# VIS4ROB-lab/covins

Measured on AMD Instinct MI355X. Metric: GBA iterations/sec, 5-agent EuRoC merged map, higher is better.
Workload: dtype f64

## Files before the change

covins_amd/csrc/nd_plan.hip:

```cpp
#include "nd_plan.hpp"

#include <algorithm>
#include <cstdint>
#include <cstdlib>
#include <queue>
#include <thread>
#include <tuple>

namespace covgpu {
namespace {

struct Builder {
  const int K;
  const bool vi;
  const int leaf_dims;
  const std::vector<std::vector<int>>& adj;
  const std::vector<int>& chain_of;
  NdHostPlan& out;
  std::vector<int> reg, deg;
  std::vector<int> side;
  std::vector<char> inS;
  int regid = 0;
  int top_mode = 0;
  double group_frac = 3.0;
// ... 109 lines not shown
              s1 += sd[pick] ? -size[pick] : size[pick]; sd[pick] ^= 1;
            }
            if (!balanced(s1, frac) || s1 == 0 || s1 == total) continue;
            if (best_w < 0 || w < best_w) { best_w = w; side_best.assign(sd.begin(), sd.end()); }
          }
      }
      if (nc <= kBruteChains) {
        if (best_w < 0) best = 2;
        side_best.assign(nc, 0);
        for (int c = 0; c < nc; ++c) side_best[c] = (char)(best >> c & 1);
      } else if (best_w < 0) {
        side_best.assign(nc, 0);
        side_best[(int)(std::max_element(size.begin(), size.end()) - size.begin())] = 1;
      }
      if (side_best[0]) for (auto& b : side_best) b ^= 1;
      for (int v : vars) side[v] = (int)side_best[side[v]];
    } else if (chains.size() >= 2) {
      nparts = (int)chains.size();
      for (int v : vars) side[v] = (int)(std::lower_bound(chains.begin(), chains.end(), chain_of[v >> 1]) - chains.begin());
    } else {
      std::vector<int> pos;
      for (int v : vars) pos.push_back(v >> 1);
      std::sort(pos.begin(), pos.end());
      pos.erase(std::unique(pos.begin(), pos.end()), pos.end());
      if (pos.size() < 2) { leaf(vars, parent); return; }
      const int m = pos[pos.size() / 2];
      for (int v : vars) side[v] = (v >> 1) >= m;
    }
    ++regid;
    for (int v : vars) { reg[v] = regid; inS[v] = 0; }
    std::priority_queue<std::tuple<int, int, int>> heap;
    for (int v : vars) {
      int d = 0;
      for (int w : adj[v]) d += (reg[w] == regid && side[w] != side[v]) ? 1 : 0;
      deg[v] = d;
      if (d) heap.push(std::make_tuple(d, 1 - (v & 1), -v));
    }
    std::vector<int> S;
    while (!heap.empty()) {
      const auto top = heap.top(); heap.pop();
      const int v = -std::get<2>(top);
      if (inS[v] || std::get<0>(top) != deg[v] || deg[v] == 0) continue;
      inS[v] = 1; S.push_back(v);
      for (int w : adj[v])
        if (reg[w] == regid && side[w] != side[v] && !inS[w] && deg[w] > 0) { if (--deg[w]) heap.push(std::make_tuple(deg[w], 1 - (w & 1), -w)); }
      deg[v] = 0;
    }
    for (size_t q = S.size(); q-- > 0;) {
      const int v = S[q];
      bool needed = false;
      for (int w : adj[v]) if (reg[w] == regid && side[w] != side[v] && !inS[w]) { needed = true; break; }
      if (!needed) { inS[v] = 0; S[q] = -1; }
    }
    S.erase(std::remove(S.begin(), S.end(), -1), S.end());
    std::vector<std::vector<int>> parts(nparts);
    for (int v : vars) if (!inS[v]) parts[side[v]].push_back(v);
    const int n = S.empty() ? parent : new_node(S, parent);
    for (auto& pt : parts) build(pt, n);
  }
};

}

static void nd_graph(int K, bool vi, int nchains, const int* chain_ptr, int npairs, const int* pair_i, const int* pair_j, int nepairs, const int* epair_i,
                     const int* epair_j, std::vector<std::vector<int>>& adj, std::vector<int>& chain_of) {
  chain_of.assign(K, 0);
  for (int c = 0; c < nchains; ++c) for (int q = chain_ptr[c]; q < chain_ptr[c + 1]; ++q) chain_of[q] = c;
  adj.assign(2 * (size_t)K, {});
  auto link = [&](int a, int b) { if (a != b) { adj[a].push_back(b); adj[b].push_back(a); } };
  for (int p = 0; p < npairs; ++p) link(2 * pair_i[p], 2 * pair_j[p]);
  for (int p = 0; p < nepairs; ++p) link(2 * epair_i[p], 2 * epair_j[p]);
  if (vi)
    for (int c = 0; c < nchains; ++c)
      for (int q = chain_ptr[c]; q < chain_ptr[c + 1]; ++q) {
        link(2 * q + 1, 2 * q);
        if (q > chain_ptr[c]) {
          const int v[4] = {2 * (q - 1), 2 * (q - 1) + 1, 2 * q, 2 * q + 1};
          for (int a = 0; a < 4; ++a) for (int b = a + 1; b < 4; ++b) link(v[a], v[b]);
        }
      }
  for (auto& a : adj) { std::sort(a.begin(), a.end()); a.erase(std::unique(a.begin(), a.end()), a.end()); }
}

static bool nd_plan_build_mode(int top_mode, double group_frac, int K, bool vi, const std::vector<std::vector<int>>& adj, const std::vector<int>& chain_of,
                               int leaf_dims, NdHostPlan& out) {
  out = NdHostPlan();
  out.K = K; out.vi = vi ? 1 : 0; out.nvar = 2 * K;
  out.vnode.assign(2 * (size_t)K, -1); out.voff.assign(2 * (size_t)K, 0); out.vord.assign(2 * (size_t)K, -1);
  if (K <= 0) return false;
  std::vector<int> all;
  for (int q = 0; q < K; ++q) { all.push_back(2 * q); if (vi) all.push_back(2 * q + 1); }
  Builder bld(K, vi, leaf_dims, adj, chain_of, out);
  bld.top_mode = top_mode; bld.group_frac = group_frac;
  bld.build(all, -1);
  const int nn = out.nnodes;
  auto is_proper_ancestor = [&](int a, int n) {
    if (out.depth[a] >= out.depth[n]) return false;
    while (out.depth[n] > out.depth[a]) n = out.parent[n];
    return n == a;
  };
  {
    std::vector<int> hgt(nn, 0);
    int nlev = 0;
    for (int n = nn - 1; n >= 0; --n) { for (int c : out.child[n]) hgt[n] = std::max(hgt[n], hgt[c] + 1); nlev = std::max(nlev, hgt[n] + 1); }
    auto panels = [](int d) { return std::max(1, (d + 255) / 256); };
    std::vector<int> levc(nlev, 1);
    for (int n = 0; n < nn; ++n) levc[hgt[n]] = std::max(levc[hgt[n]], panels(out.own_dims[n]));
    for (int l = 0; l + 1 < nlev; ++l) {
      const int m = levc[l];
      if (m < 2) continue;
      std::vector<std::pair<int, int>> moves;
      std::vector<int> extra(nn, 0);
      bool ok = true;
      for (int n = 0; n < nn && ok; ++n) {
        if (hgt[n] != l || panels(out.own_dims[n]) < m) continue;
        const int need = out.own_dims[n] - 256 * (m - 1);
        int cnt = 0, mv = 0;
        for (size_t q = out.own[n].size(); q-- > 0 && mv < need;) { mv += NdHostPlan::vdim(out.own[n][q]); ++cnt; }
        if (need > 64 || out.parent[n] < 0 || cnt >= (int)out.own[n].size()) { ok = false; break; }
        moves.emplace_back(n, cnt); extra[out.parent[n]] += mv;
      }
      for (int n = 0; n < nn && ok; ++n) if (extra[n] && panels(out.own_dims[n] + extra[n]) > levc[hgt[n]]) ok = false;
      if (!ok) continue;
      for (auto& mvp : moves) {
        const int n = mvp.first, pn = out.parent[n];
        std::vector<int> up(out.own[n].end() - mvp.second, out.own[n].end());
        out.own[n].resize(out.own[n].size() - mvp.second);
        for (int v : up) out.own[pn].push_back(v);
        for (int node : {n, pn}) {
          int off = 0, ord = 0;
          for (int v : out.own[node]) { out.vnode[v] = node; out.voff[v] = off; out.vord[v] = ord++; off += NdHostPlan::vdim(v); }
          out.own_dims[node] = off;
        }
      }
      levc[l] = m - 1;
    }
  }
  out.strct.assign(nn, {});
  out.st_dims.assign(nn, 0);
  std::vector<int> stamp(2 * (size_t)K, -1);
  for (int n = nn - 1; n >= 0; --n) {
    std::vector<int>& st = out.strct[n];
    auto add = [&](int w) { if (stamp[w] != n) { stamp[w] = n; st.push_back(w); } };
    for (int v : out.own[n])
      for (int w : adj[v]) {
        const int m = out.vnode[w];
        if (m == n) continue;
        if (is_proper_ancestor(m, n)) add(w);
        else if (!is_proper_ancestor(n, m)) return false;
      }
    for (int c : out.child[n])
      for (int w : out.strct[c]) if (out.vnode[w] != n) add(w);
    std::sort(st.begin(), st.end(), [&](int a, int b) {
      return std::make_pair(-out.depth[out.vnode[a]], out.vord[a]) < std::make_pair(-out.depth[out.vnode[b]], out.vord[b]);
    });
    int d = 0;
    for (int w : st) d += NdHostPlan::vdim(w);
    out.st_dims[n] = d;
  }
  out.level.assign(nn, 0); out.slot.assign(nn, 0);
  for (int n = nn - 1; n >= 0; --n)
    for (int c : out.child[n]) out.level[n] = std::max(out.level[n], out.level[c] + 1);
  out.nlev = 0; out.maxdepth = 0;
  for (int n = 0; n < nn; ++n) { out.nlev = std::max(out.nlev, out.level[n] + 1); out.maxdepth = std::max(out.maxdepth, out.depth[n] + 1); }
  out.lev_nodes.assign(out.nlev, {});
  for (int n = 0; n < nn; ++n) { out.slot[n] = (int)out.lev_nodes[out.level[n]].size(); out.lev_nodes[out.level[n]].push_back(n); }
  out.lev_nI.assign(out.nlev, 0); out.lev_nO.assign(out.nlev, 0); out.lev_ntot.assign(out.nlev, 0);
  for (int l = 0; l < out.nlev; ++l) {
    int mo = 0, ms = 0;
    for (int n : out.lev_nodes[l]) { mo = std::max(mo, out.own_dims[n]); ms = std::max(ms, out.st_dims[n]); }
    out.lev_nI[l] = std::max(256, ((mo + 255) / 256) * 256);
    out.lev_nO[l] = ((ms + 127) / 128) * 128;
    out.lev_ntot[l] = out.lev_nI[l] + out.lev_nO[l];
    out.front_elems += (size_t)out.lev_nodes[l].size() * out.lev_ntot[l] * out.lev_ntot[l];
  }
  for (int n = 0; n < nn; ++n) {
    const double m = out.own_dims[n], b = out.st_dims[n];
    out.flops += m * m * m / 3.0 + m * m * b + m * b * b;
  }
  return true;
}

static double nd_plan_cost(const NdHostPlan& hp) {
  double t = hp.flops / 30e12;
  for (int l = 0; l < hp.nlev; ++l) t += (hp.lev_nI[l] / 256) * 140e-6 + 40e-6;
  return t;
}

bool nd_plan_build(int K, bool vi, int nchains, const int* chain_ptr, int npairs, const int* pair_i, const int* pair_j, int nepairs,
                   const int* epair_i, const int* epair_j, int leaf_dims, NdHostPlan& out, int top_mode) {
  std::vector<std::vector<int>> adj;
  std::vector<int> chain_of;
  out = NdHostPlan();
  out.K = K; out.vi = vi ? 1 : 0; out.nvar = 2 * K;
  if (K <= 0) return false;
  nd_graph(K, vi, nchains, chain_ptr, npairs, pair_i, pair_j, nepairs, epair_i, epair_j, adj, chain_of);
  int forced = top_mode;
  if (const char* e = getenv("COVGPU_ND_TOP")) forced = atoi(e) != 0 ? 1 : 0;
  std::vector<int> modes, leaves;
  if (nchains < 3 || forced == 0 || leaf_dims >= (1 << 29)) modes = {0};
  else if (forced == 1) modes = {1};
  else modes = {0, 1};
  if (leaf_dims > 0) leaves = {leaf_dims};
  else leaves = {600, 400, 500, 900};
  std::vector<double> fracs = {3.0, 2.5};
  if (const char* e = getenv("COVGPU_ND_GROUP_FRAC")) fracs = {std::max(2.0, atof(e))};
  struct Cand { int mode, leaf; double frac; NdHostPlan hp; bool ok = false; double cost = 0; };
  std::vector<Cand> cand;
  for (int lf : leaves)
    for (int m : modes)
      for (double fr : (m == 1 ? fracs : std::vector<double>{3.0})) { cand.emplace_back(); cand.back().mode = m; cand.back().leaf = lf; cand.back().frac = fr; }
  auto run = [&](size_t i) {
    try {
      cand[i].ok = nd_plan_build_mode(cand[i].mode, cand[i].frac, K, vi, adj, chain_of, cand[i].leaf, cand[i].hp);
      if (cand[i].ok) cand[i].cost = nd_plan_cost(cand[i].hp);
    } catch (...) { cand[i].ok = false; }
  };
  if (cand.size() == 1) run(0);
  else {
    std::vector<std::thread> th;
    std::vector<char> started(cand.size(), 0);
    for (size_t i = 1; i < cand.size(); ++i) {
      try { th.emplace_back(run, i); started[i] = 1; } catch (...) { break; }
    }
    run(0);
    for (auto& t : th) t.join();
    for (size_t i = 1; i < cand.size(); ++i) if (!started[i]) run(i);
  }
  int best = -1;
  for (size_t i = 0; i < cand.size(); ++i) if (cand[i].ok && (best < 0 || cand[i].cost < cand[best].cost)) best = (int)i;
  if (best < 0) return false;
  out = std::move(cand[best].hp);
  out.top_mode = cand[best].mode; out.leaf = cand[best].leaf; out.group_frac100 = (int)(cand[best].frac * 100.0 + 0.5);
  return true;
}

double nd_shard_cost(const NdHostPlan& hp, int world) {
  const int nn = hp.nnodes;
  double chain = 0.0;
  for (int l = 0; l < hp.nlev; ++l) chain += (hp.lev_nI[l] / 256) * 140e-6 + 40e-6;
  if (hp.shard_policy == 1) {
    NdShardAcct a;
    nd_shard_account(hp, world, a);
    double busiest = 0.0;
    for (double f : a.rank_fl) busiest = std::max(busiest, f);
    constexpr double kCollLatency = 30e-6;
    return busiest / 30e12 + chain + (world > 1 ? 2.0 * (world - 1) / world * a.bytes / 150e9 + a.collectives * kCollLatency : 0.0);
  }
  double top_fl = 0.0, exch = 0.0;
  std::vector<double> rank_fl(std::max(world, 1), 0.0);
  for (int n = 0; n < nn; ++n) {
    const double m = hp.own_dims[n], b = hp.st_dims[n], fl = m * m * m / 3.0 + m * m * b + m * b * b;
    if (hp.node_rank.empty() || hp.node_rank[n] < 0) { top_fl += fl; exch += 0.5 * (m + b) * (m + b) * 8.0; }
    else rank_fl[hp.node_rank[n]] += fl;
  }
  double busiest = 0.0;
  for (double f : rank_fl) busiest = std::max(busiest, f);
  return (top_fl + busiest) / 30e12 + chain + (world > 1 ? 2.0 * (world - 1) / world * exch / 150e9 : 0.0);
}

static void nd_shard_grow(NdHostPlan& hp, int world, double top_cap_bytes, std::vector<char>& top, double top_bytes) {
  const int nn = hp.nnodes;
  hp.node_rank.assign(nn, -1);
  hp.nsub = 0;
  hp.world = world;
  std::vector<double> w(nn, 0.0), sub(nn, 0.0);
  for (int n = 0; n < nn; ++n) { const double m = hp.own_dims[n], b = hp.st_dims[n]; w[n] = m * m * m / 3.0 + m * m * b + m * b * b + 1.0; }
  for (int n = nn - 1; n >= 0; --n) { sub[n] += w[n]; if (hp.parent[n] >= 0) sub[hp.parent[n]] += sub[n]; }
  std::vector<int> cand;
  for (int n = 0; n < nn; ++n)
    if (top[n]) for (int c : hp.child[n]) if (!top[c]) cand.push_back(c);
  for (int it = 0; it < 256; ++it) {
    if (cand.empty()) break;
    std::sort(cand.begin(), cand.end(), [&](int a, int b) { return sub[a] != sub[b] ? sub[a] > sub[b] : a < b; });
    double tot = 0.0;
    for (int c : cand) tot += sub[c];
    if ((int)cand.size() >= world && sub[cand[0]] <= 1.25 * tot / world) break;
    int pick = -1;
    for (size_t q = 0; q < cand.size() && pick < 0; ++q) {
      const int c = cand[q];
      const double nb = 8.0 * (double)(hp.own_dims[c] + hp.st_dims[c]) * (double)(hp.own_dims[c] + hp.st_dims[c]);
      if (!hp.child[c].empty() && top_bytes + nb <= top_cap_bytes) pick = (int)q;
    }
    if (pick < 0) break;
    const int c = cand[pick];
    cand.erase(cand.begin() + pick);
    top[c] = 1; top_bytes += 8.0 * (double)(hp.own_dims[c] + hp.st_dims[c]) * (double)(hp.own_dims[c] + hp.st_dims[c]);
    for (int d : hp.child[c]) cand.push_back(d);
  }
  std::sort(cand.begin(), cand.end(), [&](int a, int b) { return sub[a] != sub[b] ? sub[a] > sub[b] : a < b; });
  std::vector<double> load(world, 0.0);
  std::vector<int> owner(nn, -1);
  for (int c : cand) {
    int best = 0;
    for (int r = 1; r < world; ++r) if (load[r] < load[best]) best = r;
    owner[c] = best; load[best] += sub[c];
  }
  hp.nsub = (int)cand.size();
  for (int n = 0; n < nn; ++n) {
    if (top[n]) { hp.node_rank[n] = -1; continue; }
    hp.node_rank[n] = owner[n] >= 0 ? owner[n] : hp.node_rank[hp.parent[n]];
  }
}

void nd_shard_assign(NdHostPlan& hp, int world, double top_cap_bytes) {
  hp.shard_policy = 0;
  std::vector<char> top(hp.nnodes, 0);
  double top_bytes = 0.0;
  for (int n = 0; n < hp.nnodes; ++n)
    if (hp.parent[n] < 0) { top[n] = 1; top_bytes += 8.0 * (double)hp.own_dims[n] * hp.own_dims[n]; }
  nd_shard_grow(hp, world, top_cap_bytes, top, top_bytes);
}

void nd_shard_assign_dist(NdHostPlan& hp, int world, double top_cap_bytes, int min_order) {
  hp.shard_policy = 1;
  const int nn = hp.nnodes;
  std::vector<char> top(nn, 0);
  for (int n = 0; n < nn; ++n)
    if (hp.parent[n] < 0 || hp.own_dims[n] + hp.st_dims[n] >= min_order)
      for (int a = n; a >= 0 && !top[a]; a = hp.parent[a]) top[a] = 1;
  double top_bytes = 0.0;
  for (int n = 0; n < nn; ++n) if (top[n]) top_bytes += 8.0 * (double)(hp.own_dims[n] + hp.st_dims[n]) * (double)(hp.own_dims[n] + hp.st_dims[n]);
  nd_shard_grow(hp, world, top_cap_bytes, top, top_bytes);
}

void nd_shard_account(const NdHostPlan& hp, int world, NdShardAcct& out) {
  const int nn = hp.nnodes;
  world = std::max(world, 1);
  out = NdShardAcct();
  out.rank_fl.assign(world, 0.0);
  const bool sh = !hp.node_rank.empty();
  auto is_top = [&](int n) { return !sh || hp.node_rank[n] < 0; };
  double top_own = 0.0, rhs_top = 0.0, tiles = 0.0;
  std::vector<int> toph(nn, 0);
  for (int n = nn - 1; n >= 0; --n) if (is_top(n)) for (int c : hp.child[n]) if (is_top(c)) toph[n] = std::max(toph[n], toph[c] + 1);
  std::vector<int> lev_panels;
  for (int n = 0; n < nn; ++n) {
    const double m = hp.own_dims[n], b = hp.st_dims[n];
    if (!is_top(n)) { out.rank_fl[hp.node_rank[n]] += m * m * m / 3.0 + m * m * b + m * b * b; continue; }
    top_own += m;
    const int nIr = (hp.own_dims[n] + 127) / 128, nO = (hp.st_dims[n] + 127) / 128, np = (hp.own_dims[n] + 255) / 256;
// ... 47 lines not shown
```

covins_amd/csrc/nd_plan.hpp:

```cpp
#pragma once
#include <cstdint>
#include <vector>

namespace covgpu {

struct NdHostPlan {
  int K = 0, vi = 0, nvar = 0;
  int nnodes = 0, nlev = 0, maxdepth = 0;
  std::vector<int> parent, depth, level, slot;
  std::vector<std::vector<int>> own, strct, child;
  std::vector<int> own_dims, st_dims;
  std::vector<int> vnode, voff, vord;
  std::vector<std::vector<int>> lev_nodes;
  std::vector<int> lev_nI, lev_nO, lev_ntot;
  std::vector<int> node_rank;
  int nsub = 0;
  int world = 0, shard_policy = 0;
  int top_mode = 0, leaf = 0, group_frac100 = 300;
  double flops = 0;
  size_t front_elems = 0;
  static int vdim(int v) { return (v & 1) ? 9 : 6; }
};

bool nd_plan_build(int K, bool vi, int nchains, const int* chain_ptr, int npairs, const int* pair_i, const int* pair_j, int nepairs,
                   const int* epair_i, const int* epair_j, int leaf_dims, NdHostPlan& out, int top_mode = -1);

void nd_shard_assign(NdHostPlan& hp, int world, double top_cap_bytes = 48.0 * 1048576.0);
void nd_shard_assign_dist(NdHostPlan& hp, int world, double top_cap_bytes = 48.0 * 1048576.0, int min_order = 4096);
inline int nd_tile_owner(int node, int q, int world) { return world > 0 ? (q + node) % world : 0; }
double nd_shard_cost(const NdHostPlan& hp, int world);
struct NdShardAcct { std::vector<double> rank_fl; double bytes = 0.0; int collectives = 0; };
void nd_shard_account(const NdHostPlan& hp, int world, NdShardAcct& out);
void nd_plan_remap(NdHostPlan& hp, const std::vector<int>& var_map);

}
```

covins_amd/csrc/solver.hip:

```cpp
#include <dlfcn.h>

#include <algorithm>
#include <atomic>
#include <chrono>
#include <condition_variable>
#include <memory>
#include <mutex>
#include <cmath>
#include <cstdio>
#include <cstdlib>
#include <cstring>
#include <string>
#include <thread>
#include <vector>

#include "common.hpp"
#include "nd_plan.hpp"

using namespace covgpu;

static thread_local std::string g_err;
extern "C" const char* covgpu_last_error(void) { return g_err.c_str(); }

#define HIPCHK(expr)                                                                            \
  do {                                                                                          \
    hipError_t e_ = (expr);                                                                     \
    if (e_ != hipSuccess) {                                                                     \
      g_err = std::string(#expr) + ": " + hipGetErrorString(e_);                                \
      return e_ == hipErrorOutOfMemory ? COVGPU_ERR_OUT_OF_MEMORY : COVGPU_ERR_NO_DEVICE;       \
    }                                                                                           \
  } while (0)

struct covgpu_profile_t {
  double t_build_ms = 0, t_factor_ms = 0, t_syrk_ms = 0, syrk_flops = 0;
  long n_build = 0, n_factor = 0, n_syrk = 0;
};

struct PlanCache {
  bool valid = false; int K = 0; bool vi = false; int leaf = 0;
  int top_env = -1; double frac_env = 0.0;
  std::vector<int> chain_ptr, pos_kf;
  std::vector<uint64_t> keys;
  NdHostPlan hp;
};

constexpr int COVGPU_ERR_GATE_TIMEOUT = -1000;
struct covgpu_group;
struct covgpu_context {
  int device = 0;
  hipStream_t st = nullptr;
  DevProblem P;
  bool have = false, pgo = false;
  std::vector<void*> allocs;
  size_t alloc_bytes = 0;
  double* h_scal = nullptr;
  double* h_tr = nullptr;
  double* h_box = nullptr;
  double* d_box = nullptr;
  double box_seq = 0.0;
  int profiling = 0;
  covgpu_profile_t prof;
  hipEvent_t ev[4] = {nullptr, nullptr, nullptr, nullptr};
  CholAux chol;
  PgoPlan pgo_plan;
  PlanCache plan_cache;
  NdDev nd;
  bool sharded = false;
  int rank = 0, world = 1;
  std::shared_ptr<NdHostPlan> shard_plan;
  struct Reducer* reducer = nullptr;
  double* d_red = nullptr;
  double cur_damp = 0.0;
  bool coll_failed = false;
  std::string coll_err;
  covgpu_group* group = nullptr;
  int* d_pairkey = nullptr;
  std::vector<int> h_perm;
  std::atomic<int>* peer_fail = nullptr;
};

struct Reducer {
  int rank = 0, world = 1;
  size_t calls = 0, bytes = 0;
  virtual ~Reducer() {}
  virtual int allreduce(double* dev, size_t n, int op, hipStream_t st) = 0;
  virtual void abort() {}
  virtual std::string last_error() { return "all-reduce failed"; }
};

struct GroupPtrs { double* p[16]; };
__global__ __launch_bounds__(256) void k_group_reduce(GroupPtrs g, int world, size_t n, int op, double* __restrict__ out) {
  for (size_t i = (size_t)blockIdx.x * 256 + threadIdx.x; i < n; i += (size_t)gridDim.x * 256) {
    double v = g.p[0][i];
    for (int r = 1; r < world; ++r) v = op == 0 ? v + g.p[r][i] : fmax(v, g.p[r][i]);
    out[i] = v;
  }
}
struct covgpu_group {
  int world = 1;
  std::mutex m; std::condition_variable cv; int count = 0; long gen = 0; bool broken = false;
  GroupPtrs ptrs;
  bool wait() {
    std::unique_lock<std::mutex> lk(m);
    const long g0 = gen;
    if (++count == world) { count = 0; ++gen; cv.notify_all(); return !broken; }
    cv.wait_for(lk, std::chrono::seconds(600), [&] { return gen != g0 || broken; });
    if (gen == g0) { broken = true; cv.notify_all(); return false; }
    return !broken;
  }
};
struct GroupReducer : Reducer {
  covgpu_group* g = nullptr;
  double* scratch = nullptr; size_t scratch_n = 0;
  ~GroupReducer() override { if (scratch) (void)hipFree(scratch); }
  void abort() override { std::lock_guard<std::mutex> lk(g->m); g->broken = true; g->cv.notify_all(); }
  std::string last_error() override { return "in-process group all-reduce failed (a member gave up, timed out, or the scratch allocation failed)"; }
  int allreduce(double* dev, size_t n, int op, hipStream_t st) override {
    if (n == 0) return 0;
    if (scratch_n < n) { if (scratch) (void)hipFree(scratch); if (hipMalloc((void**)&scratch, n * sizeof(double)) != hipSuccess) return 1; scratch_n = n; }
    (void)hipStreamSynchronize(st);
    { std::lock_guard<std::mutex> lk(g->m); g->ptrs.p[rank] = dev; }
    if (!g->wait()) return 1;
    hipLaunchKernelGGL(k_group_reduce, dim3((unsigned)std::min<size_t>((n + 255) / 256, 4096)), dim3(256), 0, st, g->ptrs, world, n, op, scratch);
// ... 371 lines not shown
    for (size_t h = 0; h < queue.size(); ++h) { const int u = queue[h]; for (int v : nb[u]) if (level[v] < 0) { level[v] = level[u] + 1; queue.push_back(v); } }
    return queue.back();
  };
  int pos = 0;
  for (int k = 0; k < K; ++k) {
    if (placed[k]) continue;
    const int far = bfs(k);
    for (int v : queue) level[v] = -1;
    bfs(far);
    for (int v : queue) { level[v] = -1; placed[v] = 1; perm[v] = pos; pos_kf[pos] = v; ++pos; }
    chain_ptr.push_back(pos);
  }
}

static bool host_pairs(const covgpu_problem* p, const std::vector<int>& perm, std::vector<int>& pi, std::vector<int>& pj, std::vector<int>& ei,
                       std::vector<int>& ej) {
  std::vector<long long> keys;
  for (int l = 0; l < p->num_lm; ++l)
    for (int a = p->lm_obs_ptr[l]; a < p->lm_obs_ptr[l + 1]; ++a) {
      if (p->kf_fixed[p->obs_kf[a]]) continue;
      for (int b = p->lm_obs_ptr[l]; b < p->lm_obs_ptr[l + 1]; ++b) {
        if (p->kf_fixed[p->obs_kf[b]]) continue;
        const int pa = perm[p->obs_kf[a]], pb = perm[p->obs_kf[b]];
        if (pb < pa) keys.push_back(((long long)pa << 32) | (unsigned)pb);
      }
    }
  std::sort(keys.begin(), keys.end()); keys.erase(std::unique(keys.begin(), keys.end()), keys.end());
  pi.resize(keys.size()); pj.resize(keys.size()); ei.clear(); ej.clear();
  for (size_t q = 0; q < keys.size(); ++q) { pi[q] = (int)(keys[q] >> 32); pj[q] = (int)(keys[q] & 0xffffffffll); }
  for (int e = 0; e < p->num_edge; ++e) {
    const int a = perm[p->edge_i[e]], b = perm[p->edge_j[e]];
    if (a == b) return false;
    ei.push_back(std::max(a, b)); ej.push_back(std::min(a, b));
  }
  return true;
}

static int nd_leaf_dims(int requested) {
  if (requested > 0) return requested;
  const char* e = getenv("COVGPU_ND_LEAF");
  const int v = e ? atoi(e) : 0;
  return v > 0 ? v : 0;
}
static int nd_plan_create_mode(const covgpu_options* opt, const covgpu_problem* p, int32_t leaf_dims, covgpu_nd_plan** out, int top_mode);
extern "C" int covgpu_nd_plan_create(const covgpu_options* opt, const covgpu_problem* p, int32_t leaf_dims, covgpu_nd_plan** out) { return nd_plan_create_mode(opt, p, leaf_dims, out, -1); }
static int nd_plan_create_mode(const covgpu_options* opt, const covgpu_problem* p, int32_t leaf_dims, covgpu_nd_plan** out, int top_mode) {
  return guarded([&] {
    const bool vi = !opt->visual_only;
    *out = nullptr;
    RC(validate(p, false, vi));
    std::vector<int> perm, pos_kf, chain_ptr, pi, pj, ei, ej;
    RC(build_chains(p, vi, perm, pos_kf, chain_ptr));
    if (!host_pairs(p, perm, pi, pj, ei, ej)) { g_err = "invalid problem: self edge"; return (int)COVGPU_ERR_INVALID_ARG; }
    covgpu_nd_plan* pl = new covgpu_nd_plan();
    pl->pos_kf = pos_kf;
    const auto t_pl = std::chrono::steady_clock::now();
    struct PT { std::chrono::steady_clock::time_point t0; ~PT() { if (getenv("COVGPU_PLAN_TIMING")) std::fprintf(stderr, "[covgpu] nd_plan_build %.1f ms\n", std::chrono::duration<double>(std::chrono::steady_clock::now() - t0).count() * 1e3); } } pt{t_pl};
    if (!nd_plan_build(p->num_kf, vi, (int)chain_ptr.size() - 1, chain_ptr.data(), (int)pi.size(), pi.data(), pj.data(), (int)ei.size(), ei.data(), ej.data(),
                       nd_leaf_dims(leaf_dims), pl->hp, top_mode)) {
      delete pl; g_err = "nested-dissection plan: a coupling joins two branches"; return (int)COVGPU_ERR_INVALID_ARG;
    }
    *out = pl;
    return (int)COVGPU_OK;
  });
}
extern "C" int covgpu_nd_plan_create_pgo(const covgpu_options* opt, const covgpu_problem* p, int32_t leaf_dims, covgpu_nd_plan** out) {
  (void)opt;
  return guarded([&] {
    *out = nullptr;
    RC(validate(p, true, false));
    std::vector<int> perm, pos_kf, chain_ptr;
    build_chains_pgo(p, perm, pos_kf, chain_ptr);
    std::vector<uint64_t> keys;
    for (int e = 0; e < p->num_edge; ++e) {
      const int a = perm[p->edge_i[e]], b = perm[p->edge_j[e]];
      if (a == b) { g_err = "invalid problem: self edge"; return (int)COVGPU_ERR_INVALID_ARG; }
      keys.push_back(((uint64_t)(uint32_t)std::max(a, b) << 32) | (uint32_t)std::min(a, b));
    }
    std::sort(keys.begin(), keys.end()); keys.erase(std::unique(keys.begin(), keys.end()), keys.end());
    std::vector<int> ei(keys.size()), ej(keys.size());
    for (size_t q = 0; q < keys.size(); ++q) { ei[q] = (int)(keys[q] >> 32); ej[q] = (int)(keys[q] & 0xffffffffull); }
    covgpu_nd_plan* pl = new covgpu_nd_plan();
    pl->pos_kf = pos_kf;
    if (!nd_plan_build(p->num_kf, false, (int)chain_ptr.size() - 1, chain_ptr.data(), 0, nullptr, nullptr, (int)ei.size(), ei.data(), ej.data(), nd_leaf_dims(leaf_dims), pl->hp, -1)) {
      delete pl; g_err = "nested-dissection plan: a coupling joins two branches"; return (int)COVGPU_ERR_INVALID_ARG;
    }
    *out = pl;
    return (int)COVGPU_OK;
  });
}
extern "C" void covgpu_nd_plan_destroy(covgpu_nd_plan* pl) { delete pl; }
extern "C" void covgpu_nd_plan_info(const covgpu_nd_plan* pl, int64_t* out) {
  for (int i = 0; i < 16; ++i) out[i] = 0;
  const NdHostPlan& h = pl->hp;
  out[0] = h.nnodes; out[1] = h.nlev; out[2] = h.maxdepth;
  for (int n = 0; n < h.nnodes; ++n) {
    out[3] += (int64_t)h.own[n].size(); out[4] += (int64_t)h.strct[n].size();
    out[7] = std::max<int64_t>(out[7], h.own_dims[n]); out[8] = std::max<int64_t>(out[8], h.st_dims[n]);
    if (h.parent[n] < 0) out[9] = std::max<int64_t>(out[9], h.own_dims[n]);
  }
  out[5] = (int64_t)h.front_elems; out[6] = (int64_t)h.flops;
  out[10] = h.top_mode; out[11] = h.leaf; out[12] = h.group_frac100;
  out[13] = h.shard_policy;
}
extern "C" int32_t covgpu_nd_plan_rank_flops(const covgpu_nd_plan* pl, double* out) {
  const NdHostPlan& h = pl->hp;
  const int world = h.node_rank.empty() ? 1 : std::max(h.world, 1);
  NdShardAcct a;
  nd_shard_account(h, world, a);
  for (int r = 0; r < world; ++r) out[r] = a.rank_fl[r];
  return world;
}
extern "C" void covgpu_nd_plan_exchange(const covgpu_nd_plan* pl, int64_t* out) {
  const NdHostPlan& h = pl->hp;
  const int world = h.node_rank.empty() ? 1 : std::max(h.world, 1);
  NdShardAcct a;
  nd_shard_account(h, world, a);
  out[0] = (int64_t)a.bytes; out[1] = a.collectives; out[2] = world; out[3] = h.shard_policy;
}
extern "C" void covgpu_nd_plan_arrays(const covgpu_nd_plan* pl, int32_t* parent, int32_t* level, int32_t* own_ptr, int32_t* own_var, int32_t* st_ptr,
                                      int32_t* st_var) {
  const NdHostPlan& h = pl->hp;
  int o = 0, s = 0;
  auto ir = [&](int v) { return 2 * pl->pos_kf[v >> 1] + (v & 1); };
  for (int n = 0; n < h.nnodes; ++n) {
    parent[n] = h.parent[n]; level[n] = h.level[n]; own_ptr[n] = o; st_ptr[n] = s;
    for (int v : h.own[n]) own_var[o++] = ir(v);
    for (int v : h.strct[n]) st_var[s++] = ir(v);
  }
  own_ptr[h.nnodes] = o; st_ptr[h.nnodes] = s;
}

extern "C" int32_t covgpu_shard_plan(const covgpu_options* opt, const covgpu_problem* p, int32_t world, covgpu_nd_plan** plan_out, int32_t* lm_rank,
                                     int32_t* imu_rank, int32_t* edge_rank) {
  *plan_out = nullptr;
  if (world < 1) return 0;
  int policy = opt->shard_policy;
  if (const char* e = getenv("COVGPU_SHARD_POLICY")) policy = atoi(e);
  if (policy != 0 && policy != 1) { g_err = "covgpu_shard_plan: shard_policy must be 0 or 1"; return 0; }
  covgpu_nd_plan* pl = nullptr;
  {
    const char* e_tree = getenv("COVGPU_SHARD_TREE");
    const char* e_cap = getenv("COVGPU_SHARD_CAP_MIB");
    std::vector<int> modes = e_tree ? std::vector<int>{atoi(e_tree) != 0 ? 1 : 0} : std::vector<int>{0, 1};
    std::vector<double> caps = e_cap ? std::vector<double>{atof(e_cap)} : std::vector<double>{48.0, 512.0};
    double best_cost = 0.0;
    for (int mode : modes) {
      covgpu_nd_plan* cand = nullptr;
      if (nd_plan_create_mode(opt, p, 0, &cand, mode) != COVGPU_OK) continue;
      for (double cap : caps) {
        NdHostPlan trial = cand->hp;
        if (policy == 1) nd_shard_assign_dist(trial, world, cap * 1048576.0);
        else nd_shard_assign(trial, world, cap * 1048576.0);
        if (trial.nsub == 0) continue;
        const double cost = nd_shard_cost(trial, world);
        if (pl == nullptr || cost < best_cost) {
          if (pl == nullptr) { pl = new covgpu_nd_plan(); pl->pos_kf = cand->pos_kf; }
          pl->hp = std::move(trial); best_cost = cost;
        }
      }
      delete cand;
    }
    if (pl == nullptr) return 0;
  }
  NdHostPlan& hp = pl->hp;
  const bool vi = !opt->visual_only;
  std::vector<int> perm(p->num_kf);
// ... 178 lines not shown
  RC(dev_upload(c, &P.edge_sqrt_info, p->edge_sqrt_info, (size_t)36 * P.E));
  RC(dev_upload(c, &P.edge_loss_a, p->edge_loss_a, (size_t)P.E));
  RC(dev_upload(c, &P.perm, perm.data(), K)); RC(dev_upload(c, &P.pos_kf, pos_kf.data(), K));
  RC(dev_upload(c, &P.chain_ptr, chain_ptr.data(), chain_ptr.size()));
  RC(dev_upload(c, &P.pos_chain_end, chain_end.data(), K));
  RC(dev_alloc(c, &P.bred, (size_t)P.n));
  RC(dev_alloc(c, &P.bp, (size_t)2 * P.npad));
  const size_t Kv = vi ? K : 0;
  RC(dev_alloc(c, &P.Ad, 81 * Kv)); RC(dev_alloc(c, &P.Ae, 81 * Kv));
  RC(dev_alloc(c, &P.Bp, 54 * Kv)); RC(dev_alloc(c, &P.Bs, 54 * Kv)); RC(dev_alloc(c, &P.Bn, 54 * Kv));
  {
    std::vector<int> cbeg(P.K);
    for (int ch = 0; ch < P.nchains; ++ch) for (int q = chain_ptr[ch]; q < chain_ptr[ch + 1]; ++q) cbeg[q] = chain_ptr[ch];
    RC(dev_upload(c, &P.pos_chain_begin, cbeg.data(), cbeg.size()));
    HIPCHK(hipStreamSynchronize(c->st));
  }
  RC(dev_alloc(c, &P.grad, (size_t)P.N)); RC(dev_alloc(c, &P.hdiag, (size_t)P.N));
  RC(dev_alloc(c, &P.HllInv, (size_t)6 * P.L));
  RC(dev_alloc(c, &P.gn, (size_t)P.N)); RC(dev_alloc(c, &P.step, (size_t)P.N)); RC(dev_alloc(c, &P.vtmp, (size_t)P.N));
  HIPCHK(hipMemsetAsync(P.gn, 0, (size_t)P.N * sizeof(double), c->st)); HIPCHK(hipMemsetAsync(P.step, 0, (size_t)P.N * sizeof(double), c->st));
  HIPCHK(hipMemsetAsync(P.vtmp, 0, (size_t)P.N * sizeof(double), c->st));
  RC(dev_alloc(c, &P.scal, (size_t)SC_COUNT)); RC(dev_alloc(c, &P.flag, (size_t)4));
  RC(dev_alloc(c, &P.tr, (size_t)TR_COUNT));
  P.scal_r = P.scal; P.flag_r = P.flag;
  P.part_imu = 8192; P.part_edge = P.part_imu + ((P.I + 3) / 4) * 4; P.part_vec = P.part_edge + (P.E + 63) / 64;
  P.part_n = P.part_vec + 8192;
  RC(dev_alloc(c, &P.part, (size_t)SC_COUNT * P.part_n));
  HIPCHK(hipMemsetAsync(P.part, 0, (size_t)SC_COUNT * P.part_n * sizeof(double), c->st));
  RC(dev_alloc(c, &P.imuAd, 2 * 81 * Kv)); RC(dev_alloc(c, &P.imuBs, 2 * 54 * Kv));
  RC(dev_alloc(c, &P.imuCd, 3 * 36 * Kv)); RC(dev_alloc(c, &P.imuG, 2 * 30 * Kv));
  RC(dev_alloc(c, &P.edgeOut, (size_t)132 * P.E));
  {
    std::vector<int> kptr(P.K + 1, 0), kent(2 * (size_t)P.E);
    for (int e = 0; e < P.E; ++e) {
      if (p->edge_i[e] == p->edge_j[e]) { g_err = "invalid problem: self edge"; return COVGPU_ERR_INVALID_ARG; }
      kptr[p->edge_i[e] + 1]++; kptr[p->edge_j[e] + 1]++;
    }
    for (int k = 0; k < P.K; ++k) kptr[k + 1] += kptr[k];
    { std::vector<int> cur(kptr.begin(), kptr.end() - 1);
      for (int e = 0; e < P.E; ++e) { kent[cur[p->edge_i[e]]++] = 2 * e; kent[cur[p->edge_j[e]]++] = 2 * e + 1; } }
    struct PE { int i, j, ent; };
    std::vector<PE> pe(P.E);
    for (int e = 0; e < P.E; ++e) {
      const int a = perm[p->edge_i[e]], b = perm[p->edge_j[e]];
      pe[e] = (a > b) ? PE{a, b, 2 * e} : PE{b, a, 2 * e + 1};
    }
    std::stable_sort(pe.begin(), pe.end(), [](const PE& x, const PE& y) { return x.i != y.i ? x.i < y.i : x.j < y.j; });
    std::vector<int> eptr, ei, ej, eent(P.E);
    for (int q = 0; q < P.E; ++q) {
      if (q == 0 || pe[q].i != pe[q - 1].i || pe[q].j != pe[q - 1].j) { eptr.push_back(q); ei.push_back(pe[q].i); ej.push_back(pe[q].j); }
      eent[q] = pe[q].ent;
    }
    eptr.push_back(P.E);
    P.nepairs = (int)ei.size();
    RC(dev_upload(c, &P.kf_edge_ptr, kptr.data(), kptr.size())); RC(dev_upload(c, &P.kf_edge_ent, kent.data(), kent.size()));
    RC(dev_upload(c, &P.epair_ptr, eptr.data(), eptr.size())); RC(dev_upload(c, &P.epair_i, ei.data(), ei.size()));
    RC(dev_upload(c, &P.epair_j, ej.data(), ej.size())); RC(dev_upload(c, &P.epair_ent, eent.data(), eent.size()));
    HIPCHK(hipStreamSynchronize(c->st));
    tm("IMU, edges, vectors");
    if (use_nd) {
      NdHostPlan nhp;
      if (c->sharded) {
        if ((int)c->shard_plan->K != P.K || (c->shard_plan->vi != 0) != vi) { g_err = "sharded solve: the problem does not match the shard plan"; return COVGPU_ERR_INVALID_ARG; }
        nhp = *c->shard_plan;
        std::vector<int> to_pos(2 * (size_t)P.K);
        for (int k = 0; k < P.K; ++k) { to_pos[2 * k] = 2 * perm[k]; to_pos[2 * k + 1] = 2 * perm[k] + 1; }
        nd_plan_remap(nhp, to_pos);
      } else {
        const bool one_front = e_dense && e_dense[0] == '1';
        const int leaf = one_front ? 0x3fffffff : nd_leaf_dims(0);
        std::vector<uint64_t> keys(h_pair_i.size() + ei.size());
        {
          std::vector<uint64_t> ka(h_pair_i.size()), kb(ei.size());
          for (size_t q = 0; q < ka.size(); ++q) ka[q] = ((uint64_t)(uint32_t)h_pair_i[q] << 32) | (uint32_t)h_pair_j[q];
          for (size_t q = 0; q < kb.size(); ++q) kb[q] = ((uint64_t)(uint32_t)ei[q] << 32) | (uint32_t)ej[q];
          if (!std::is_sorted(ka.begin(), ka.end())) std::sort(ka.begin(), ka.end());
          std::merge(ka.begin(), ka.end(), kb.begin(), kb.end(), keys.begin());
          keys.erase(std::unique(keys.begin(), keys.end()), keys.end());
        }
        PlanCache& pc = c->plan_cache;
        const char *e_top = getenv("COVGPU_ND_TOP"), *e_frac = getenv("COVGPU_ND_GROUP_FRAC");
        const int top_env = e_top ? (atoi(e_top) != 0 ? 1 : 0) : -1;
        const double frac_env = e_frac ? std::max(2.0, atof(e_frac)) : 0.0;
        const bool hit = pc.valid && pc.K == P.K && pc.vi == vi && pc.leaf == leaf && pc.top_env == top_env && pc.frac_env == frac_env && pc.chain_ptr == chain_ptr && pc.pos_kf == pos_kf &&
                         std::includes(pc.keys.begin(), pc.keys.end(), keys.begin(), keys.end());
        if (hit) nhp = pc.hp;
        else {
          if (!nd_plan_build(P.K, vi, P.nchains, chain_ptr.data(), (int)h_pair_i.size(), h_pair_i.data(), h_pair_j.data(), P.nepairs, ei.data(), ej.data(), leaf, nhp)) {
            g_err = "nested-dissection plan: a coupling joins two branches"; return COVGPU_ERR_INVALID_ARG;
          }
          pc.valid = true; pc.K = P.K; pc.vi = vi; pc.leaf = leaf; pc.top_env = top_env; pc.frac_env = frac_env; pc.chain_ptr = chain_ptr; pc.pos_kf = pos_kf; pc.keys.swap(keys); pc.hp = nhp;
        }
      }
      if (nhp.maxdepth > 64) { g_err = "nested-dissection plan: tree deeper than 64 levels"; return COVGPU_ERR_INVALID_ARG; }
      tm("nested-dissection plan");
      NdDev& nd = c->nd;
      nd_tables(nhp, pos_kf.data(), P.D, c->rank, nd);
      tm("front tables");
      P.nd = 1; P.nd_nnodes = nd.nnodes; P.nd_nlev = (int)nd.lev.size(); P.nd_maxd = nhp.maxdepth;
      nd.ntop = (int)nd.h_top_g.size();
      RC(dev_upload(c, &P.nd_vnode, nd.h_vnode.data(), nd.h_vnode.size())); RC(dev_upload(c, &P.nd_voff, nd.h_voff.data(), nd.h_voff.size()));
      RC(dev_upload(c, &P.nd_vord, nd.h_vord.data(), nd.h_vord.size()));
      if (c->sharded) RC(dev_upload(c, &P.nd_vown, nd.h_vown.data(), nd.h_vown.size()));
      RC(dev_upload(c, &P.nd_ndepth, nd.h_ndepth.data(), nd.h_ndepth.size())); RC(dev_upload(c, &P.nd_nI, nd.h_nI.data(), nd.h_nI.size()));
      RC(dev_upload(c, &P.nd_ntab, nd.h_ntab.data(), nd.h_ntab.size()));
      RC(dev_upload(c, &P.nd_abase, nd.h_abase.data(), nd.h_abase.size())); RC(dev_upload(c, &P.nd_fidx, nd.h_fidx.data(), nd.h_fidx.size()));
      RC(dev_upload(c, &nd.own_dims, nd.h_own_dims.data(), nd.h_own_dims.size())); RC(dev_upload(c, &nd.st_dims, nd.h_st_dims.data(), nd.h_st_dims.size()));
      RC(dev_upload(c, &nd.own_g, nd.h_own_g.data(), nd.h_own_g.size())); RC(dev_upload(c, &nd.st_g, nd.h_st_g.data(), nd.h_st_g.size()));
      RC(dev_upload(c, &nd.gidx, nd.h_gidx.data(), nd.h_gidx.size()));
      RC(dev_upload(c, &nd.tree_fill, nd.h_tree_fill.empty() ? (const int*)nullptr : nd.h_tree_fill.data(), std::max<size_t>(nd.h_tree_fill.size(), 1)));
      RC(dev_upload(c, &nd.cptr, nd.h_cptr.data(), nd.h_cptr.size())); RC(dev_upload(c, &nd.cidx, nd.h_cidx.data(), nd.h_cidx.size()));
      RC(dev_upload(c, &nd.cptr2, nd.h_cptr2.data(), nd.h_cptr2.size())); RC(dev_upload(c, &nd.cidx2, nd.h_cidx2.data(), nd.h_cidx2.size()));
      RC(dev_upload(c, &nd.inv_off, nd.h_inv_off.data(), nd.h_inv_off.size())); RC(dev_upload(c, &nd.inv, nd.h_inv.data(), nd.h_inv.size()));
      RC(dev_upload(c, &nd.rhs_node, nd.h_rhs_node.data(), nd.h_rhs_node.size()));
      RC(dev_upload(c, &nd.ext, nd.h_ext.data(), nd.h_ext.size()));
      auto up_or_zero = [&](int** dst, const std::vector<int>& h, size_t least) { return dev_upload(c, dst, h.empty() ? (const int*)nullptr : h.data(), std::max(h.size(), least)); };
      RC(up_or_zero(&nd.extw, nd.h_extw, 8)); RC(up_or_zero(&nd.extc, nd.h_extc, 6)); RC(up_or_zero(&nd.extc2, nd.h_extc2, 6));
      RC(up_or_zero(&nd.extr, nd.h_extr, kExtRec));
      RC(dev_upload(c, &nd.bb_off, nd.h_bb_off.data(), nd.h_bb_off.size()));
      RC(dev_upload(c, &nd.bb, nd.h_bb.data(), std::max<size_t>(nd.h_bb.size(), 1)));
      RC(dev_upload(c, &nd.top_var, nd.h_top_var.data(), nd.h_top_var.size())); RC(dev_upload(c, &nd.top_r, nd.h_top_r.data(), nd.h_top_r.size()));
      RC(dev_upload(c, &nd.top_g, nd.h_top_g.data(), nd.h_top_g.size()));
      for (NdLevel& L : nd.lev) { RC(dev_upload(c, &L.live, L.live_h.data(), L.live_h.size())); RC(dev_upload(c, &L.plist, L.plist_h.data(), L.plist_h.size())); }
      RC(dev_alloc(c, &P.nd_M, nd.M_elems + nd.rhs_elems));
      P.nd_rhs = P.nd_M + nd.M_elems;
      RC(dev_alloc(c, &P.nd_Linv, nd.linv_elems));
      RC(dev_alloc(c, &P.nd_dummy, (size_t)64));
      launch_nd_init(P, nd, c->st);
      c->chol.tri_clear();
      HIPCHK(hipStreamSynchronize(c->st));
      tm("table upload, front allocation");
      if (c->sharded) {
        P.shard = 1;
        std::vector<double> vw((size_t)P.N, 1.0);
        for (int k = 0; k < P.K; ++k) {
          const int op = nd.h_vown[2 * perm[k]], os = nd.h_vown[2 * perm[k] + 1];
          const double wp = op == 1 ? 1.0 : (op == 2 && c->rank == 0 ? 1.0 : 0.0), ws = os == 1 ? 1.0 : (os == 2 && c->rank == 0 ? 1.0 : 0.0);
          for (int r = 0; r < 6; ++r) vw[(size_t)P.D * k + r] = wp;
          for (int r = 6; r < P.D; ++r) vw[(size_t)P.D * k + r] = ws;
        }
        RC(dev_upload(c, &P.vw, vw.data(), vw.size()));
        RC(dev_alloc(c, &c->d_red, (size_t)SC_COUNT + 2 * (size_t)c->world));
        nd.n_top_tiles = (int)(nd.h_top_tiles.size() / 3);
        if (nd.dist) {
          RC(up_or_zero(&nd.dist_ent, nd.h_dist_ent, 4)); RC(up_or_zero(&nd.dist_tri, nd.h_dist_tri, 1));
          RC(dev_alloc(c, &nd.dist_buf, std::max<size_t>(nd.dist_buf_elems, 1)));
          for (NdLevel& L : nd.lev) {
            L.dt_dev.assign(L.dt_cnt.size(), nullptr);
            for (size_t q = 0; q < L.dt_cnt.size(); ++q) if (L.dt_cnt[q] > 0) L.dt_dev[q] = nd.dist_tri + L.dt_first[q];
          }
        } else {
          RC(dev_upload(c, &nd.top_tiles, nd.h_top_tiles.data(), nd.h_top_tiles.size()));
          RC(dev_alloc(c, &nd.top_pack, (size_t)nd.n_top_tiles * kTile * kTile + nd.rhs_top + 2 * (size_t)nd.ntop));
        }
        RC(dev_alloc(c, &P.scal_r, (size_t)SC_COUNT)); RC(dev_alloc(c, &P.flag_r, (size_t)4));
      }
      HIPCHK(hipStreamSynchronize(c->st));
      if (opt->verbose) {
        int panels = 0;
        for (const NdLevel& L : nd.lev) panels += L.nI / 256;
        std::printf("[covgpu] multifrontal plan: %d fronts in %d levels (%d serial 256-column panels), %.2e flops, fronts %.2f GB%s\n", nd.nnodes,
                    (int)nd.lev.size(), panels, nhp.flops, nd.M_elems * 8e-9, c->sharded ? " (this rank's share)" : "");
      }
    } else {
      RC(dev_alloc(c, &P.Sred, (size_t)P.npad * P.npad));
      RC(dev_alloc(c, &P.Linv, (size_t)(P.npad / kTile) * kTile * kTile));
    }
  }
  if (pgo && P.E && !pgo_nd) {
    PgoHostPlan hp;
    const char* dense = getenv("COVGPU_PGO_DENSE");
    if (!(dense && dense[0] == '1') && pgo_plan_analyse(P.K, P.E, p->edge_i, p->edge_j, hp)) {
      PgoPlan& plan = c->pgo_plan;
      std::vector<int> idxb;
// ... 1554 lines not shown
```

Before: 291.9.

## Add cost-model-driven level amalgamation to the nested-dissection front tree

Adds a greedy amalgamation pass that merges whole tree levels into their parents whenever a refined cost model predicts a saving, which cuts the number of level-synchronous factorization steps. The per-level cost model is recalibrated: panel cost now depends on the widest front and on whether the front is bordered, and the flop rate is raised. Merging trades fewer level launches and less per-level latency for larger fronts with more dense flops and memory. It is on by default, but disabled for PGO and the sharded-plan API, and the plan cache key now includes the merge setting.

```diff
diff --git a/covins_amd/csrc/nd_plan.hip b/covins_amd/csrc/nd_plan.hip
--- a/covins_amd/csrc/nd_plan.hip
+++ b/covins_amd/csrc/nd_plan.hip
@@ -215,8 +215,11 @@
   for (auto& a : adj) { std::sort(a.begin(), a.end()); a.erase(std::unique(a.begin(), a.end()), a.end()); }
 }
 
+static bool nd_plan_finish(const std::vector<std::vector<int>>& adj, NdHostPlan& out);
+static bool nd_amalgamate(const std::vector<std::vector<int>>& adj, NdHostPlan& out);
+
 static bool nd_plan_build_mode(int top_mode, double group_frac, int K, bool vi, const std::vector<std::vector<int>>& adj, const std::vector<int>& chain_of,
-                               int leaf_dims, NdHostPlan& out) {
+                               int leaf_dims, bool merge, NdHostPlan& out) {
   out = NdHostPlan();
   out.K = K; out.vi = vi ? 1 : 0; out.nvar = 2 * K;
   out.vnode.assign(2 * (size_t)K, -1); out.voff.assign(2 * (size_t)K, 0); out.vord.assign(2 * (size_t)K, -1);
@@ -227,11 +230,6 @@
   bld.top_mode = top_mode; bld.group_frac = group_frac;
   bld.build(all, -1);
   const int nn = out.nnodes;
-  auto is_proper_ancestor = [&](int a, int n) {
-    if (out.depth[a] >= out.depth[n]) return false;
-    while (out.depth[n] > out.depth[a]) n = out.parent[n];
-    return n == a;
-  };
   {
     std::vector<int> hgt(nn, 0);
     int nlev = 0;
@@ -269,9 +267,20 @@
       levc[l] = m - 1;
     }
   }
+  if (!nd_plan_finish(adj, out)) return false;
+  return merge ? nd_amalgamate(adj, out) : true;
+}
+
+static bool nd_plan_finish(const std::vector<std::vector<int>>& adj, NdHostPlan& out) {
+  const int nn = out.nnodes;
+  auto is_proper_ancestor = [&](int a, int n) {
+    if (out.depth[a] >= out.depth[n]) return false;
+    while (out.depth[n] > out.depth[a]) n = out.parent[n];
+    return n == a;
+  };
   out.strct.assign(nn, {});
   out.st_dims.assign(nn, 0);
-  std::vector<int> stamp(2 * (size_t)K, -1);
+  std::vector<int> stamp((size_t)out.nvar, -1);
   for (int n = nn - 1; n >= 0; --n) {
     std::vector<int>& st = out.strct[n];
     auto add = [&](int w) { if (stamp[w] != n) { stamp[w] = n; st.push_back(w); } };
@@ -299,6 +308,7 @@
   out.lev_nodes.assign(out.nlev, {});
   for (int n = 0; n < nn; ++n) { out.slot[n] = (int)out.lev_nodes[out.level[n]].size(); out.lev_nodes[out.level[n]].push_back(n); }
   out.lev_nI.assign(out.nlev, 0); out.lev_nO.assign(out.nlev, 0); out.lev_ntot.assign(out.nlev, 0);
+  out.front_elems = 0; out.flops = 0;
   for (int l = 0; l < out.nlev; ++l) {
     int mo = 0, ms = 0;
     for (int n : out.lev_nodes[l]) { mo = std::max(mo, out.own_dims[n]); ms = std::max(ms, out.st_dims[n]); }
@@ -314,14 +324,102 @@
   return true;
 }
 
-static double nd_plan_cost(const NdHostPlan& hp) {
-  double t = hp.flops / 30e12;
-  for (int l = 0; l < hp.nlev; ++l) t += (hp.lev_nI[l] / 256) * 140e-6 + 40e-6;
+constexpr double kLevelS = 34e-6, kPanelBorderS = 45e-6, kPanelRootS = 49e-6, kPanelColS = 0.155e-6, kFlopRate = 40e12;
+constexpr double kMergeMarginS = 20e-6;
+
+static double nd_level_cost(int widest_own, bool bordered) {
+  double t = kLevelS;
+  for (int c = 0; c < std::max(widest_own, 1); c += 256) t += (bordered ? kPanelBorderS : kPanelRootS) + kPanelColS * std::min(256, std::max(widest_own, 1) - c);
   return t;
 }
+static double nd_front_flops(double m, double b) { return m * m * m / 3.0 + m * m * b + m * b * b; }
+static double nd_chain_cost(const NdHostPlan& hp) {
+  double t = 0.0;
+  for (int l = 0; l < hp.nlev; ++l) {
+    int mo = 1;
+    for (int n : hp.lev_nodes[l]) mo = std::max(mo, hp.own_dims[n]);
+    t += nd_level_cost(mo, hp.lev_nO[l] > 0);
+  }
+  return t;
+}
+static double nd_plan_cost(const NdHostPlan& hp) { return hp.flops / kFlopRate + nd_chain_cost(hp); }
+
+bool nd_merge_enabled() {
+  const char* e = getenv("COVGPU_ND_MERGE");
+  return e == nullptr || atoi(e) != 0;
+}
+
+static void nd_merge_level(NdHostPlan& out, int l) {
+  const int nn = out.nnodes;
+  std::vector<int> hgt(nn, 0), id(nn, -1);
+  for (int n = nn - 1; n >= 0; --n) for (int c : out.child[n]) hgt[n] = std::max(hgt[n], hgt[c] + 1);
+  std::vector<std::vector<int>> front(nn);
+  int kept = 0;
+  for (int n = 0; n < nn; ++n) {
+    const int p = out.parent[n];
+    if (hgt[n] == l && p >= 0 && hgt[p] == l + 1) front[p].insert(front[p].end(), out.own[n].begin(), out.own[n].end());
+    else id[n] = kept++;
+  }
+  NdHostPlan t;
+  t.K = out.K; t.vi = out.vi; t.nvar = out.nvar; t.nnodes = kept;
+  t.vnode.assign(out.vnode.size(), -1); t.voff.assign(out.voff.size(), 0); t.vord.assign(out.vord.size(), -1);
+  t.parent.resize(kept); t.depth.resize(kept); t.own.resize(kept); t.own_dims.resize(kept); t.child.assign(kept, {});
+  for (int n = 0; n < nn; ++n) {
+    if (id[n] < 0) continue;
+    const int m = id[n];
+    int p = out.parent[n];
+    if (p >= 0 && id[p] < 0) p = out.parent[p];
+    t.parent[m] = p < 0 ? -1 : id[p];
+    t.depth[m] = p < 0 ? 0 : t.depth[id[p]] + 1;
+    if (p >= 0) t.child[id[p]].push_back(m);
+    t.own[m].swap(front[n]);
+    t.own[m].insert(t.own[m].end(), out.own[n].begin(), out.own[n].end());
+    int off = 0, ord = 0;
+    for (int v : t.own[m]) { t.vnode[v] = m; t.voff[v] = off; t.vord[v] = ord++; off += NdHostPlan::vdim(v); }
+    t.own_dims[m] = off;
+  }
+  out = std::move(t);
+}
+
+static double nd_merge_trial_cost(const NdHostPlan& hp, int l) {
+  const int nn = hp.nnodes;
+  std::vector<int> add(nn, 0), mo(hp.nlev - 1, 1);
+  std::vector<char> merged(nn, 0), bordered(hp.nlev - 1, 0);
+  double flops = hp.flops;
+  for (int n = 0; n < nn; ++n) {
+    const int p = hp.parent[n];
+    if (hp.level[n] != l || p < 0 || hp.level[p] != l + 1) continue;
+    merged[n] = 1; add[p] += hp.own_dims[n];
+    flops -= nd_front_flops(hp.own_dims[n], hp.st_dims[n]);
+  }
+  for (int n = 0; n < nn; ++n) {
+    if (merged[n]) continue;
+    if (add[n]) flops += nd_front_flops(hp.own_dims[n] + add[n], hp.st_dims[n]) - nd_front_flops(hp.own_dims[n], hp.st_dims[n]);
+    const int h = hp.level[n] > l ? hp.level[n] - 1 : hp.level[n];
+    mo[h] = std::max(mo[h], hp.own_dims[n] + add[n]);
+    if (hp.st_dims[n] > 0) bordered[h] = 1;
+  }
+  double t = flops / kFlopRate;
+  for (int h = 0; h + 1 < hp.nlev; ++h) t += nd_level_cost(mo[h], bordered[h] != 0);
+  return t;
+}
+
+static bool nd_amalgamate(const std::vector<std::vector<int>>& adj, NdHostPlan& out) {
+  for (;;) {
+    double best_cost = nd_plan_cost(out) - kMergeMarginS;
+    int best = -1;
+    for (int l = 0; l + 1 < out.nlev; ++l) {
+      const double c = nd_merge_trial_cost(out, l);
+      if (c < best_cost) { best_cost = c; best = l; }
+    }
+    if (best < 0) return true;
+    nd_merge_level(out, best);
+    if (!nd_plan_finish(adj, out)) return false;
+  }
+}
 
 bool nd_plan_build(int K, bool vi, int nchains, const int* chain_ptr, int npairs, const int* pair_i, const int* pair_j, int nepairs,
-                   const int* epair_i, const int* epair_j, int leaf_dims, NdHostPlan& out, int top_mode) {
+                   const int* epair_i, const int* epair_j, int leaf_dims, NdHostPlan& out, int top_mode, bool allow_merge) {
   std::vector<std::vector<int>> adj;
   std::vector<int> chain_of;
   out = NdHostPlan();
@@ -330,6 +428,7 @@
   nd_graph(K, vi, nchains, chain_ptr, npairs, pair_i, pair_j, nepairs, epair_i, epair_j, adj, chain_of);
   int forced = top_mode;
   if (const char* e = getenv("COVGPU_ND_TOP")) forced = atoi(e) != 0 ? 1 : 0;
+  const bool merge = allow_merge && leaf_dims <= 0 && top_mode < 0 && nd_merge_enabled();
   std::vector<int> modes, leaves;
   if (nchains < 3 || forced == 0 || leaf_dims >= (1 << 29)) modes = {0};
   else if (forced == 1) modes = {1};
@@ -345,7 +444,7 @@
       for (double fr : (m == 1 ? fracs : std::vector<double>{3.0})) { cand.emplace_back(); cand.back().mode = m; cand.back().leaf = lf; cand.back().frac = fr; }
   auto run = [&](size_t i) {
     try {
-      cand[i].ok = nd_plan_build_mode(cand[i].mode, cand[i].frac, K, vi, adj, chain_of, cand[i].leaf, cand[i].hp);
+      cand[i].ok = nd_plan_build_mode(cand[i].mode, cand[i].frac, K, vi, adj, chain_of, cand[i].leaf, merge, cand[i].hp);
       if (cand[i].ok) cand[i].cost = nd_plan_cost(cand[i].hp);
     } catch (...) { cand[i].ok = false; }
   };
@@ -370,15 +469,14 @@
 
 double nd_shard_cost(const NdHostPlan& hp, int world) {
   const int nn = hp.nnodes;
-  double chain = 0.0;
-  for (int l = 0; l < hp.nlev; ++l) chain += (hp.lev_nI[l] / 256) * 140e-6 + 40e-6;
+  const double chain = nd_chain_cost(hp);
   if (hp.shard_policy == 1) {
     NdShardAcct a;
     nd_shard_account(hp, world, a);
     double busiest = 0.0;
     for (double f : a.rank_fl) busiest = std::max(busiest, f);
     constexpr double kCollLatency = 30e-6;
-    return busiest / 30e12 + chain + (world > 1 ? 2.0 * (world - 1) / world * a.bytes / 150e9 + a.collectives * kCollLatency : 0.0);
+    return busiest / kFlopRate + chain + (world > 1 ? 2.0 * (world - 1) / world * a.bytes / 150e9 + a.collectives * kCollLatency : 0.0);
   }
   double top_fl = 0.0, exch = 0.0;
   std::vector<double> rank_fl(std::max(world, 1), 0.0);
@@ -389,7 +487,7 @@
   }
   double busiest = 0.0;
   for (double f : rank_fl) busiest = std::max(busiest, f);
-  return (top_fl + busiest) / 30e12 + chain + (world > 1 ? 2.0 * (world - 1) / world * exch / 150e9 : 0.0);
+  return (top_fl + busiest) / kFlopRate + chain + (world > 1 ? 2.0 * (world - 1) / world * exch / 150e9 : 0.0);
 }
 
 static void nd_shard_grow(NdHostPlan& hp, int world, double top_cap_bytes, std::vector<char>& top, double top_bytes) {
diff --git a/covins_amd/csrc/nd_plan.hpp b/covins_amd/csrc/nd_plan.hpp
--- a/covins_amd/csrc/nd_plan.hpp
+++ b/covins_amd/csrc/nd_plan.hpp
@@ -23,7 +23,8 @@
 };
 
 bool nd_plan_build(int K, bool vi, int nchains, const int* chain_ptr, int npairs, const int* pair_i, const int* pair_j, int nepairs,
-                   const int* epair_i, const int* epair_j, int leaf_dims, NdHostPlan& out, int top_mode = -1);
+                   const int* epair_i, const int* epair_j, int leaf_dims, NdHostPlan& out, int top_mode = -1, bool allow_merge = true);
+bool nd_merge_enabled();
 
 void nd_shard_assign(NdHostPlan& hp, int world, double top_cap_bytes = 48.0 * 1048576.0);
 void nd_shard_assign_dist(NdHostPlan& hp, int world, double top_cap_bytes = 48.0 * 1048576.0, int min_order = 4096);
diff --git a/covins_amd/csrc/solver.hip b/covins_amd/csrc/solver.hip
--- a/covins_amd/csrc/solver.hip
+++ b/covins_amd/csrc/solver.hip
@@ -39,6 +39,7 @@
 struct PlanCache {
   bool valid = false; int K = 0; bool vi = false; int leaf = 0;
   int top_env = -1; double frac_env = 0.0;
+  bool merge_env = true;
   std::vector<int> chain_ptr, pos_kf;
   std::vector<uint64_t> keys;
   NdHostPlan hp;
@@ -576,7 +577,7 @@
     for (size_t q = 0; q < keys.size(); ++q) { ei[q] = (int)(keys[q] >> 32); ej[q] = (int)(keys[q] & 0xffffffffull); }
     covgpu_nd_plan* pl = new covgpu_nd_plan();
     pl->pos_kf = pos_kf;
-    if (!nd_plan_build(p->num_kf, false, (int)chain_ptr.size() - 1, chain_ptr.data(), 0, nullptr, nullptr, (int)ei.size(), ei.data(), ej.data(), nd_leaf_dims(leaf_dims), pl->hp, -1)) {
+    if (!nd_plan_build(p->num_kf, false, (int)chain_ptr.size() - 1, chain_ptr.data(), 0, nullptr, nullptr, (int)ei.size(), ei.data(), ej.data(), nd_leaf_dims(leaf_dims), pl->hp, -1, false)) {
       delete pl; g_err = "nested-dissection plan: a coupling joins two branches"; return (int)COVGPU_ERR_INVALID_ARG;
     }
     *out = pl;
@@ -921,14 +922,15 @@
         const char *e_top = getenv("COVGPU_ND_TOP"), *e_frac = getenv("COVGPU_ND_GROUP_FRAC");
         const int top_env = e_top ? (atoi(e_top) != 0 ? 1 : 0) : -1;
         const double frac_env = e_frac ? std::max(2.0, atof(e_frac)) : 0.0;
-        const bool hit = pc.valid && pc.K == P.K && pc.vi == vi && pc.leaf == leaf && pc.top_env == top_env && pc.frac_env == frac_env && pc.chain_ptr == chain_ptr && pc.pos_kf == pos_kf &&
+        const bool merge_env = nd_merge_enabled() && !pgo;
+        const bool hit = pc.valid && pc.K == P.K && pc.vi == vi && pc.leaf == leaf && pc.top_env == top_env && pc.frac_env == frac_env && pc.merge_env == merge_env && pc.chain_ptr == chain_ptr && pc.pos_kf == pos_kf &&
                          std::includes(pc.keys.begin(), pc.keys.end(), keys.begin(), keys.end());
         if (hit) nhp = pc.hp;
         else {
-          if (!nd_plan_build(P.K, vi, P.nchains, chain_ptr.data(), (int)h_pair_i.size(), h_pair_i.data(), h_pair_j.data(), P.nepairs, ei.data(), ej.data(), leaf, nhp)) {
+          if (!nd_plan_build(P.K, vi, P.nchains, chain_ptr.data(), (int)h_pair_i.size(), h_pair_i.data(), h_pair_j.data(), P.nepairs, ei.data(), ej.data(), leaf, nhp, -1, !pgo)) {
             g_err = "nested-dissection plan: a coupling joins two branches"; return COVGPU_ERR_INVALID_ARG;
           }
-          pc.valid = true; pc.K = P.K; pc.vi = vi; pc.leaf = leaf; pc.top_env = top_env; pc.frac_env = frac_env; pc.chain_ptr = chain_ptr; pc.pos_kf = pos_kf; pc.keys.swap(keys); pc.hp = nhp;
+          pc.valid = true; pc.K = P.K; pc.vi = vi; pc.leaf = leaf; pc.top_env = top_env; pc.frac_env = frac_env; pc.merge_env = merge_env; pc.chain_ptr = chain_ptr; pc.pos_kf = pos_kf; pc.keys.swap(keys); pc.hp = nhp;
         }
       }
       if (nhp.maxdepth > 64) { g_err = "nested-dissection plan: tree deeper than 64 levels"; return COVGPU_ERR_INVALID_ARG; }
```

After: 301.1, median of 6. +3.2%, better.
